# youssefg7/dl-sound-classification

Hardware: AMD Instinct MI355X
Metric: training clips/sec (EnvNet-v2, ESC-50 shape) (higher is better)
Workload: dtype bf16; 1 GPU; EnvNet-v2 train step (BC-mix, fwd, soft-CE, bwd, clip, Adam), ESC-50 shape; global_batch=256, per_gpu_batch=256, clip_samples=220500, parallelism=dp1, model=envnet_v2

## Files before the change

dl-sound-classification_amd/csrc/conv1ch.hip:

```cpp
#include "common.h"

namespace {

constexpr int C1_C = 32, C1_K = 8;
constexpr int C1_BW = 128;
constexpr int C1_SLOTS = C1_BW + C1_K - 1;
constexpr int C1_PSB = 80;
constexpr int C1_HMAX = 64;
constexpr int C1_OLD = C1_BW + 1;
constexpr int C1_LD = (C1_SLOTS * 4 + 255) / 256;

struct C1Args {
  const bf16* dy;
  const float* w;
  bf16* dx;
  int n, oh, ow, h, wd, nchunk;
};

__global__ __launch_bounds__(256) void conv1ch_dgrad_kernel(C1Args g) {
  __shared__ __attribute__((aligned(16))) char rows[2][C1_SLOTS * C1_PSB];
  __shared__ __attribute__((aligned(16))) float outs[C1_HMAX * C1_OLD];
  const int t = threadIdx.x, lane = t & 63, wave = t >> 6;
  const int b = blockIdx.x / g.nchunk;
  const int w0 = (blockIdx.x - b * g.nchunk) * C1_BW;

  for (int i = t; i < C1_HMAX * C1_OLD; i += 256) outs[i] = 0.f;

  bf16x8 bw[16];
  const int ky = lane & 31;
#pragma unroll
  for (int ks = 0; ks < 16; ++ks) {
    const int kx = ks >> 1, co0 = 16 * (ks & 1) + 8 * (lane >> 5);
#pragma unroll
    for (int j = 0; j < 8; ++j)
      bw[ks][j] = ky < C1_K ? (bf16)g.w[((co0 + j) * C1_K + ky) * C1_K + kx] : (bf16)0.f;
  }

  auto slot_of = [](int q, int& s, int& c) __attribute__((always_inline)) {
    const int gq = q >> 3, j = q & 7;
    s = (gq >> 2) * 8 + (gq & 3) + 4 * (j >> 2);
    c = j & 3;
  };
  const bf16* dyb = g.dy + (int64_t)b * g.oh * g.ow * C1_C;
  auto load_row = [&](int r, uint4 (&reg)[C1_LD]) __attribute__((always_inline)) {
    const bf16* src = dyb + (int64_t)r * g.ow * C1_C;
#pragma unroll
    for (int i = 0; i < C1_LD; ++i) {
      int s, c;
      slot_of(t + 256 * i, s, c);
      const int px = w0 - (C1_K - 1) + s;
      uint4 v = make_uint4(0, 0, 0, 0);
      if (r < g.oh && s < C1_SLOTS && px >= 0 && px < g.ow)
        v = *reinterpret_cast<const uint4*>(src + px * C1_C + c * 8);
      reg[i] = v;
    }
  };
  auto store_row = [&](char* dst, const uint4 (&reg)[C1_LD]) __attribute__((always_inline)) {
#pragma unroll
    for (int i = 0; i < C1_LD; ++i) {
      int s, c;
      slot_of(t + 256 * i, s, c);
      if (s < C1_SLOTS) *reinterpret_cast<uint4*>(dst + s * C1_PSB + c * 16) = reg[i];
    }
  };
  const int m = lane & 31, half = lane >> 5;
  auto compute_row = [&](int r) __attribute__((always_inline)) {
    const char* cur = rows[r & 1];
    f32x16 acc;
#pragma unroll
    for (int i = 0; i < 16; ++i) acc[i] = 0.f;
#pragma unroll
    for (int ks = 0; ks < 16; ++ks) {
      const int slot = 32 * wave + m - (ks >> 1) + (C1_K - 1);
      const bf16x8 a = *reinterpret_cast<const bf16x8*>(cur + slot * C1_PSB + (16 * (ks & 1) + 8 * half) * 2);
      acc = __builtin_amdgcn_mfma_f32_32x32x16_bf16(a, bw[ks], acc, 0, 0, 0);
    }
    if (ky < C1_K) {
      float* o = outs + (r + ky) * C1_OLD + 32 * wave + 4 * half;
#pragma unroll
      for (int i = 0; i < 16; ++i) o[(i & 3) + 8 * (i >> 2)] += acc[i];
    }
  };

  uint4 ra[C1_LD], rb[C1_LD];
  load_row(0, ra);
  load_row(1, rb);
  store_row(rows[0], ra);
  __syncthreads();
  for (int r = 0; r < g.oh; r += 2) {
    load_row(r + 2, ra);
    compute_row(r);
    store_row(rows[(r + 1) & 1], rb);
    __syncthreads();
    if (r + 1 >= g.oh) break;
    load_row(r + 3, rb);
    compute_row(r + 1);
    store_row(rows[r & 1], ra);
    __syncthreads();
  }

  bf16* dxb = g.dx + (int64_t)b * g.h * g.wd;
  for (int q = t; q < g.h * (C1_BW / 4); q += 256) {
    const int y = q / (C1_BW / 4), x4 = (q - y * (C1_BW / 4)) * 4;
    const int x = w0 + x4;
    if (x >= g.wd) continue;
    const float* o = outs + y * C1_OLD + x4;
    if (x + 4 <= g.wd) {
      bf16x4 v = {(bf16)o[0], (bf16)o[1], (bf16)o[2], (bf16)o[3]};
      *reinterpret_cast<bf16x4*>(dxb + (int64_t)y * g.wd + x) = v;
    } else {
      for (int i = 0; x + i < g.wd; ++i) dxb[(int64_t)y * g.wd + x + i] = (bf16)o[i];
    }
  }
}

}

extern "C" int mia_conv1ch_dgrad(const void* dy, const float* w, void* dx, int32_t n, int32_t oh, int32_t ow,
                                 mia_stream_t stream) {
  MIA_CHECK_ARG(dy && w && dx && n > 0 && oh > 0 && ow > 0, "conv1ch_dgrad: bad arguments");
  const int h = oh + C1_K - 1, wd = ow + C1_K - 1;
  MIA_CHECK_ARG(h <= C1_HMAX, "conv1ch_dgrad: at most %d output rows (got %d)", C1_HMAX, h);
  MIA_CHECK_ARG(wd % 4 == 0, "conv1ch_dgrad: output width must be a multiple of 4 (got %d)", wd);
  MIA_CHECK_ARG((reinterpret_cast<uintptr_t>(dy) | reinterpret_cast<uintptr_t>(dx)) % 16 == 0,
                "conv1ch_dgrad: dy/dx must be 16-byte aligned");
  MIA_CHECK_ARG((int64_t)oh * ow * C1_C < (1ll << 31), "conv1ch_dgrad: clip too large for 32-bit indexing");
  C1Args a{reinterpret_cast<const bf16*>(dy), w, reinterpret_cast<bf16*>(dx), n, oh, ow, h, wd,
           (int)cdiv(wd, C1_BW)};
  const int64_t blocks = (int64_t)n * a.nchunk;
  MIA_CHECK_ARG(blocks < (1ll << 31), "conv1ch_dgrad: grid too large");
  conv1ch_dgrad_kernel<<<(unsigned)blocks, 256, 0, as_stream(stream)>>>(a);
  MIA_LAUNCH_CHECK("conv1ch_dgrad");
  return 0;
}
```

dl-sound-classification_amd/csrc/dgemm.hip:

```cpp
#include <type_traits>

#include "gemm_common.h"
#include "../../include/miaudio_optim.h"

namespace {

using namespace mgemm;

constexpr int NT = 256;



typedef __attribute__((address_space(3))) void* lds_vp;
typedef const __attribute__((address_space(1))) void* glb_vp;

__device__ __forceinline__ void tile_sqsum_store(double* dst, double v, double* red) {
  v = wave_sum_d(v);
  __syncthreads();
  if ((threadIdx.x & 63) == 0) red[threadIdx.x >> 6] = v;
  __syncthreads();
  if (threadIdx.x == 0) {
    double s = 0.0;
#pragma unroll
    for (int w = 0; w < NT / 64; ++w) s += red[w];
    *dst = s;
  }
}

__global__ __launch_bounds__(NT) void tile_sqsum_kernel(const float* __restrict__ c, int64_t ldc, int64_t M, int64_t N,
                                                        int nbn, double* __restrict__ out) {
  const int bm = blockIdx.x / nbn, bn = blockIdx.x - (blockIdx.x / nbn) * nbn;
  const int64_t m0 = (int64_t)bm * 128, n0 = (int64_t)bn * 128;
  float sq = 0.f;
  for (int e = threadIdx.x; e < 128 * 128; e += NT) {
    const int64_t m = m0 + e / 128, n = n0 + e % 128;
    if (m < M && n < N) {
      const float v = c[m * ldc + n];
      sq = fmaf(v, v, sq);
    }
  }
  __shared__ double red[NT / 64];
  tile_sqsum_store(out + blockIdx.x, (double)sq, red);
}

__device__ __forceinline__ int dkc_swz(int r) { return (r >> 1) & 7; }

template <int L>
struct DLoader {
  const bf16* src[4];
  int64_t step;
  __device__ __forceinline__ void init(const bf16* base, int64_t ld, int64_t rows_or_cols, int64_t r0, int64_t kbeg,
                                       int wave, int lane) {
#pragma unroll
    for (int i = 0; i < 4; ++i) {
      const int j = wave * 4 + i;
      if constexpr (L == MIA_LAYOUT_KC) {
        const int r = 8 * j + (lane >> 3);
        const int c = (lane & 7) ^ dkc_swz(r);
        int64_t row = r0 + r;
        if (row >= rows_or_cols) row = rows_or_cols - 1;
        src[i] = base + row * ld + kbeg + c * 8;
      } else {
        const int kr = 4 * j + (lane >> 4);
        const int p = lane & 15;
        const int c = 2 * ((p >> 1) ^ (kr & 3)) + (p & 1);
        int64_t col = r0 + c * 8;
        if (col + 8 > rows_or_cols) col = rows_or_cols - 8;
        src[i] = base + (kbeg + kr) * ld + col;
      }
    }
    step = L == MIA_LAYOUT_KC ? 64 : 64 * ld;
  }
  __device__ __forceinline__ void issue(char* tile, int wave) {
#pragma unroll
    for (int i = 0; i < 4; ++i) {
      __builtin_amdgcn_global_load_lds((glb_vp)src[i], (lds_vp)(tile + (wave * 4 + i) * 1024), 16, 0, 0);
      src[i] += step;
    }
  }
};

template <int L>
__device__ __forceinline__ bf16x8 dfrag(const char* tile, int rbase, int ks, int lane) {
  if constexpr (L == MIA_LAYOUT_KC) {
    const int rr = rbase + (lane & 31);
    const int c = 2 * ks + (lane >> 5);
    return *reinterpret_cast<const bf16x8*>(tile + rr * 128 + ((c ^ dkc_swz(rr)) * 16));
  } else {
    const int i16 = lane & 15, gq = lane >> 4;
    const int col = rbase + 16 * (gq & 1) + 4 * (i16 & 3);
    const int kr = ks * 16 + 8 * (gq >> 1) + (i16 >> 2);
    const char* p0 = tile + kr * 256 + (((col >> 4) ^ (kr & 3)) * 32) + (col & 15) * 2;
    const s16x4 lo = __builtin_amdgcn_ds_read_tr16_b64_v4i16((MIA_LDS s16x4*)(p0));
    const s16x4 hi = __builtin_amdgcn_ds_read_tr16_b64_v4i16((MIA_LDS s16x4*)(p0 + 4 * 256));
    typedef short s16x8 __attribute__((ext_vector_type(8)));
    const s16x8 cc = {lo[0], lo[1], lo[2], lo[3], hi[0], hi[1], hi[2], hi[3]};
    return __builtin_bit_cast(bf16x8, cc);
  }
}


constexpr int TILE = 128 * 64 * 2;

template <int NS, class R>
__device__ __forceinline__ void dgemm_update_tile(const DArgs& g, const UpdateEpi<R>& o, char* smem) {
  constexpr int L = MIA_LAYOUT_RC;
  const int t = threadIdx.x, lane = t & 63;
  const int wave = __builtin_amdgcn_readfirstlane(t >> 6);
  const int wm = wave >> 1, wn = wave & 1;
  const int nwg = g.nbm * g.nbn;
  const int orig = blockIdx.x;
  const int xcd = orig % 8, q8 = nwg / 8, r8 = nwg % 8;
  const int wgid = (xcd < r8 ? xcd * (q8 + 1) : r8 * (q8 + 1) + (xcd - r8) * q8) + orig / 8;
  const int bm = wgid % g.nbm, bn = wgid / g.nbm;
  const int64_t m0 = (int64_t)bm * 128, n0 = (int64_t)bn * 128;
  const int nk = (int)(g.K / 64);

  DLoader<L> la;
  DLoader<L> lb;
  la.init(g.a, g.lda, g.M, m0, 0, wave, lane);
  lb.init(g.b, g.ldb, g.N, n0, 0, wave, lane);

  f32x16 acc[2][2];
#pragma unroll
  for (int i = 0; i < 2; ++i)
#pragma unroll
    for (int j = 0; j < 2; ++j)
#pragma unroll
      for (int r = 0; r < 16; ++r) acc[i][j][r] = 0.f;

  f32x4 pv[2][4], av[2][4], bv[2][4];
  const int acol = (lane & 31) * 4;
  auto fetch = [&](int it0, int b) {
#pragma unroll
    for (int u = 0; u < 4; ++u) {
      const int64_t off = (m0 + wave * 32 + (it0 + u) * 2 + (lane >> 5)) * o.ld + n0 + acol;
      pv[b][u] = __builtin_nontemporal_load(reinterpret_cast<const f32x4*>(o.p + off));
      if constexpr (NS > 0) av[b][u] = __builtin_nontemporal_load(reinterpret_cast<const f32x4*>(o.s0 + off));
      if constexpr (NS > 1) bv[b][u] = __builtin_nontemporal_load(reinterpret_cast<const f32x4*>(o.s1 + off));
    }
  };
  fetch(0, 0);

  if (nk > 0) {
    la.issue(smem, wave);
    lb.issue(smem + TILE, wave);
  }
  for (int kt = 0; kt < nk; ++kt) {
    char* cur = smem + (kt & 1) * 2 * TILE;
    if (kt + 1 < nk) {
      char* nxt = smem + ((kt + 1) & 1) * 2 * TILE;
      la.issue(nxt, wave);
      lb.issue(nxt + TILE, wave);
      asm volatile("s_waitcnt vmcnt(8)" ::: "memory");
    } else {
      asm volatile("s_waitcnt vmcnt(0)" ::: "memory");
    }
    __builtin_amdgcn_s_barrier();
    const char* As = cur;
    const char* Bs = cur + TILE;
#pragma unroll
    for (int ks = 0; ks < 4; ++ks) {
      bf16x8 fa[2], fb[2];
#pragma unroll
      for (int i = 0; i < 2; ++i) fa[i] = dfrag<L>(As, wm * 64 + i * 32, ks, lane);
#pragma unroll
      for (int j = 0; j < 2; ++j) fb[j] = dfrag<L>(Bs, wn * 64 + j * 32, ks, lane);
#pragma unroll
      for (int i = 0; i < 2; ++i)
#pragma unroll
        for (int j = 0; j < 2; ++j) acc[i][j] = __builtin_amdgcn_mfma_f32_32x32x16_bf16(fa[i], fb[j], acc[i][j], 0, 0, 0);
    }
    asm volatile("s_waitcnt lgkmcnt(0)" ::: "memory");
    __builtin_amdgcn_s_barrier();
  }

  float* tile = reinterpret_cast<float*>(smem);
#pragma unroll
  for (int i = 0; i < 2; ++i)
#pragma unroll
    for (int j = 0; j < 2; ++j)
#pragma unroll
      for (int r = 0; r < 16; ++r) {
        const int row = wm * 64 + i * 32 + (r & 3) + 8 * (r >> 2) + 4 * (lane >> 5);
        const int col = wn * 64 + j * 32 + (lane & 31);
        tile[row * 128 + (col ^ (((row >> 2) & 1) << 5))] = acc[i][j][r];
      }
  __syncthreads();
  const float coef = o.coef[0];
  const bool first = o.first != 0;
#pragma unroll
  for (int grp = 0; grp < 4; ++grp) {
    const int b = grp & 1;
    if (grp + 1 < 4) fetch((grp + 1) * 4, b ^ 1);
#pragma unroll
    for (int u = 0; u < 4; ++u) {
      const int row = wave * 32 + (grp * 4 + u) * 2 + (lane >> 5);
      const int64_t off = (m0 + row) * o.ld + n0 + acol;
      const f32x4 gv = *reinterpret_cast<const f32x4*>(tile + row * 128 + (acol ^ (((row >> 2) & 1) << 5)));
      f32x4 p4 = pv[b][u], a4 = {0.f, 0.f, 0.f, 0.f}, b4 = a4;
      if constexpr (NS > 0) a4 = av[b][u];
      if constexpr (NS > 1) b4 = bv[b][u];
#pragma unroll
      for (int e = 0; e < 4; ++e) {
        float sa = a4[e], sb = b4[e];
        p4[e] = mopt::apply<NS>(o.rule, coef, first, p4[e], gv[e], sa, sb);
        a4[e] = sa;
        b4[e] = sb;
      }
      __builtin_nontemporal_store(p4, reinterpret_cast<f32x4*>(o.p + off));
      if constexpr (NS > 0) __builtin_nontemporal_store(a4, reinterpret_cast<f32x4*>(o.s0 + off));
      if constexpr (NS > 1) __builtin_nontemporal_store(b4, reinterpret_cast<f32x4*>(o.s1 + off));
      if (o.shadow) {
        const bf16x4 h4 = {(bf16)p4[0], (bf16)p4[1], (bf16)p4[2], (bf16)p4[3]};
        __builtin_nontemporal_store(h4, reinterpret_cast<bf16x4*>(o.shadow + off));
      }
    }
  }
}

template <int NS, class R>
__global__ __launch_bounds__(NT) void dgemm_optim_kernel(DArgs g, UpdateEpi<R> o) {
  __shared__ __attribute__((aligned(1024))) char smem[4 * TILE];
  dgemm_update_tile<NS>(g, o, smem);
}

template <int LA, int LB, bool ADAM = false>
__global__ __launch_bounds__(NT) void dgemm_kernel(DArgs g) {
  __shared__ __attribute__((aligned(1024))) char smem[4 * TILE];
  if constexpr (ADAM) {
    dgemm_update_tile<2>(g, g.upd, smem);
    return;
  }
  const int t = threadIdx.x, lane = t & 63;
  const int wave = __builtin_amdgcn_readfirstlane(t >> 6);
  const int wm = wave >> 1, wn = wave & 1;
  const int nwg = g.nbm * g.nbn;
  const int orig = blockIdx.x;
  const int xcd = orig % 8, q8 = nwg / 8, r8 = nwg % 8;
  const int wgid = (xcd < r8 ? xcd * (q8 + 1) : r8 * (q8 + 1) + (xcd - r8) * q8) + orig / 8;
  int bm, bn;
  if (g.nfast) {
    const int gsize = g.gm * g.nbn;
    const int grp = wgid / gsize, rem = wgid - grp * gsize;
    const int gme = min(g.gm, g.nbm - grp * g.gm);
    bm = grp * g.gm + rem % gme;
    bn = rem / gme;
  } else {
    bm = wgid % g.nbm;
    bn = wgid / g.nbm;
  }
  const int64_t m0 = (int64_t)bm * 128, n0 = (int64_t)bn * 128;
  const int z = blockIdx.y;
  const int64_t kbeg = (int64_t)z * g.kper;
  int64_t kend = kbeg + g.kper;
  if (kend > g.K) kend = g.K;
  const int nk = kend > kbeg ? (int)((kend - kbeg) / 64) : 0;

  DLoader<LA> la;
  DLoader<LB> lb;
  la.init(g.a, g.lda, g.M, m0, kbeg, wave, lane);
  lb.init(g.b, g.ldb, g.N, n0, kbeg, wave, lane);

  f32x16 acc[2][2];
#pragma unroll
  for (int i = 0; i < 2; ++i)
#pragma unroll
    for (int j = 0; j < 2; ++j)
#pragma unroll
      for (int r = 0; r < 16; ++r) acc[i][j][r] = 0.f;

  if (nk > 0) {
    la.issue(smem, wave);
    lb.issue(smem + TILE, wave);
  }
  for (int kt = 0; kt < nk; ++kt) {
    char* cur = smem + (kt & 1) * 2 * TILE;
    if (kt + 1 < nk) {
      char* nxt = smem + ((kt + 1) & 1) * 2 * TILE;
      la.issue(nxt, wave);
      lb.issue(nxt + TILE, wave);
      asm volatile("s_waitcnt vmcnt(8)" ::: "memory");
    } else {
      asm volatile("s_waitcnt vmcnt(0)" ::: "memory");
    }
    __builtin_amdgcn_s_barrier();
    const char* As = cur;
    const char* Bs = cur + TILE;
#pragma unroll
    for (int ks = 0; ks < 4; ++ks) {
      bf16x8 fa[2], fb[2];
#pragma unroll
      for (int i = 0; i < 2; ++i) fa[i] = dfrag<LA>(As, wm * 64 + i * 32, ks, lane);
#pragma unroll
      for (int j = 0; j < 2; ++j) fb[j] = dfrag<LB>(Bs, wn * 64 + j * 32, ks, lane);
#pragma unroll
      for (int i = 0; i < 2; ++i)
#pragma unroll
        for (int j = 0; j < 2; ++j) acc[i][j] = __builtin_amdgcn_mfma_f32_32x32x16_bf16(fa[i], fb[j], acc[i][j], 0, 0, 0);
    }
    asm volatile("s_waitcnt lgkmcnt(0)" ::: "memory");
    __builtin_amdgcn_s_barrier();
  }

  const bool plain = g.mode != 0 ||
                     (g.split == 1 && g.e.dtype == MIA_F32 && g.e.act == MIA_ACT_NONE && !g.e.bias &&
                      !g.e.accumulate && !g.e.rm_inner && g.e.alpha == 1.f && m0 + 128 <= g.M && n0 + 128 <= g.N &&
                      (g.e.ldc & 3) == 0 && ((reinterpret_cast<uintptr_t>(g.e.ptr)) & 15) == 0);
  if (plain) {
    float sq = 0.f;
    if (g.e.sqsum) {
#pragma unroll
      for (int i = 0; i < 2; ++i)
#pragma unroll
        for (int j = 0; j < 2; ++j)
#pragma unroll
          for (int r = 0; r < 16; ++r) sq = fmaf(acc[i][j][r], acc[i][j][r], sq);
    }
    if (g.mode == 1) {
      tile_sqsum_store(g.e.sqsum + (int64_t)bm * g.nbn + bn, (double)sq, reinterpret_cast<double*>(smem));
      return;
    }
    float* tile = reinterpret_cast<float*>(smem);
#pragma unroll
    for (int i = 0; i < 2; ++i)
#pragma unroll
      for (int j = 0; j < 2; ++j)
#pragma unroll
        for (int r = 0; r < 16; ++r) {
          const int row = wm * 64 + i * 32 + (r & 3) + 8 * (r >> 2) + 4 * (lane >> 5);
          const int col = wn * 64 + j * 32 + (lane & 31);
          tile[row * 128 + (col ^ (((row >> 2) & 1) << 5))] = acc[i][j][r];
        }
    __syncthreads();
    float* out = reinterpret_cast<float*>(g.e.ptr);
#pragma unroll 4
    for (int it = 0; it < 16; ++it) {
      const int row = wave * 32 + it * 2 + (lane >> 5);
      const int col = (lane & 31) * 4;
      const f32x4 v = *reinterpret_cast<const f32x4*>(tile + row * 128 + (col ^ (((row >> 2) & 1) << 5)));
      __builtin_nontemporal_store(v, reinterpret_cast<f32x4*>(out + (m0 + row) * g.e.ldc + n0 + col));
    }
    if (g.e.sqsum) tile_sqsum_store(g.e.sqsum + (int64_t)bm * g.nbn + bn, (double)sq, reinterpret_cast<double*>(smem));
    return;
  }
  const bool save = g.e.act == MIA_ACT_GELU_SAVE || g.e.act == MIA_ACT_GELU_SAVE_D;
  const bool save_d = g.e.act == MIA_ACT_GELU_SAVE_D;
  const bool drop = g.e.rm_inner && g.e.rm_offset == MIA_RM_DROP && g.e.rm_istride == 1 &&
                    (g.e.act == MIA_ACT_NONE || g.e.act == MIA_ACT_RELU);
  const bool plain16 = g.split == 1 && g.e.dtype == MIA_BF16 &&
                       (g.e.act == MIA_ACT_NONE || g.e.act == MIA_ACT_RELU || g.e.act == MIA_ACT_GELU ||
                        (save && g.e.aux_dtype == MIA_BF16 && (g.e.ldaux & 7) == 0 &&
                         ((reinterpret_cast<uintptr_t>(g.e.aux)) & 15) == 0)) &&
                       !g.e.accumulate && (!g.e.rm_inner || drop) &&
                       g.e.alpha == 1.f && m0 + 128 <= g.M && n0 + 128 <= g.N && (g.e.ldc & 7) == 0 &&
                       ((reinterpret_cast<uintptr_t>(g.e.ptr)) & 15) == 0;
  if (plain16) {
    float* tile = reinterpret_cast<float*>(smem);
#pragma unroll
    for (int i = 0; i < 2; ++i)
#pragma unroll
      for (int j = 0; j < 2; ++j)
#pragma unroll
        for (int r = 0; r < 16; ++r) {
          const int row = wm * 64 + i * 32 + (r & 3) + 8 * (r >> 2) + 4 * (lane >> 5);
          const int col = wn * 64 + j * 32 + (lane & 31);
          tile[row * 128 + (col ^ (((row >> 2) & 1) << 5))] = acc[i][j][r];
        }
    __syncthreads();
    const int col = (lane & 15) * 8;
    float bv[8];
#pragma unroll
    for (int c = 0; c < 8; ++c) bv[c] = g.e.bias ? g.e.bias[n0 + col + c] : 0.f;
    const bool relu = g.e.act == MIA_ACT_RELU, gelu = g.e.act == MIA_ACT_GELU || save;
    bf16* out = reinterpret_cast<bf16*>(g.e.ptr);
    auto pack = [](const float* f) {
      uint32_t w4[4];
#pragma unroll
      for (int q = 0; q < 4; ++q) {
        w4[q] = pk_bf16(f[2 * q], f[2 * q + 1]);
      }
      return make_uint4(w4[0], w4[1], w4[2], w4[3]);
    };
#pragma unroll 4
    for (int it = 0; it < 8; ++it) {
      const int row = wave * 32 + it * 4 + (lane >> 4);
      const int sw = ((row >> 2) & 1) << 5;
      const f32x4 a = *reinterpret_cast<const f32x4*>(tile + row * 128 + (col ^ sw));
      const f32x4 b = *reinterpret_cast<const f32x4*>(tile + row * 128 + ((col + 4) ^ sw));
      float v[8] = {a[0], a[1], a[2], a[3], b[0], b[1], b[2], b[3]};
#pragma unroll
      for (int c = 0; c < 8; ++c) v[c] += bv[c];
      if (save) {
        float d[8];
#pragma unroll
        for (int c = 0; c < 8; ++c) d[c] = save_d ? gelu_erf_grad((float)(bf16)v[c]) : v[c];
        *reinterpret_cast<uint4*>(reinterpret_cast<bf16*>(const_cast<char*>(g.e.aux)) + (m0 + row) * g.e.ldaux +
                                  n0 + col) = pack(d);
      }
#pragma unroll
      for (int c = 0; c < 8; ++c) v[c] = relu ? fmaxf(v[c], 0.f) : (gelu ? gelu_erf(v[c]) : v[c]);
      int64_t prow = m0 + row;
      if (drop) {
        const int64_t x = prow % g.e.rm_inner;
        if (x >= g.e.rm_outer) continue;
        prow = (prow / g.e.rm_inner) * g.e.rm_outer + x;
      }
      *reinterpret_cast<uint4*>(out + prow * g.e.ldc + n0 + col) = pack(v);
    }
    return;
  }

  float* stage = reinterpret_cast<float*>(smem) + wave * (32 * 33);
  double sqg = 0.0;
#pragma unroll
  for (int i = 0; i < 2; ++i)
#pragma unroll
    for (int j = 0; j < 2; ++j) {
#pragma unroll
      for (int r = 0; r < 16; ++r)
        stage[((r & 3) + 8 * (r >> 2) + 4 * (lane >> 5)) * 33 + (lane & 31)] = acc[i][j][r];
      __syncthreads();
      const int row = lane >> 1, c0 = (lane & 1) * 16;
      const int64_t m = m0 + wm * 64 + i * 32 + row;
      const int64_t nb = n0 + wn * 64 + j * 32 + c0;
      if (m < g.M && nb < g.N) {
        float v[16];
#pragma unroll
        for (int c = 0; c < 16; ++c) v[c] = stage[row * 33 + c0 + c];
        if (g.split > 1) {
          float* dst = g.ws + ((int64_t)z * g.M + m) * g.N + nb;
          if (nb + 16 <= g.N && (g.N & 3) == 0) {
#pragma unroll
            for (int q = 0; q < 4; ++q)
              reinterpret_cast<float4*>(dst)[q] = make_float4(v[4 * q], v[4 * q + 1], v[4 * q + 2], v[4 * q + 3]);
          } else {
            for (int c = 0; c < 16; ++c)
              if (nb + c < g.N) dst[c] = v[c];
          }
        } else {
          epi_store16(g.e, m, nb, g.N, v);
          if (g.e.sqsum) {
            float sq = 0.f;
            for (int c = 0; c < 16; ++c)
              if (nb + c < g.N) sq = fmaf(v[c], v[c], sq);
            sqg += sq;
          }
        }
      }
      __syncthreads();
    }
  if (g.e.sqsum && g.split == 1)
    tile_sqsum_store(g.e.sqsum + (int64_t)bm * g.nbn + bn, sqg, reinterpret_cast<double*>(smem));
}

template <int LA, int LB>
hipError_t dgemm_launch2(const DArgs& d, hipStream_t s) {
  dim3 grid((unsigned)(d.nbm * d.nbn), (unsigned)d.split);
  dgemm_kernel<LA, LB><<<grid, NT, 0, s>>>(d);
  return hipGetLastError();
}

hipError_t dgemm_launch(const DArgs& d, int la, int lb, hipStream_t s) {
  if (la == MIA_LAYOUT_KC && lb == MIA_LAYOUT_KC) return dgemm_launch2<MIA_LAYOUT_KC, MIA_LAYOUT_KC>(d, s);
  if (la == MIA_LAYOUT_KC) return dgemm_launch2<MIA_LAYOUT_KC, MIA_LAYOUT_RC>(d, s);
  if (lb == MIA_LAYOUT_KC) return dgemm_launch2<MIA_LAYOUT_RC, MIA_LAYOUT_KC>(d, s);
  return dgemm_launch2<MIA_LAYOUT_RC, MIA_LAYOUT_RC>(d, s);
}

DArgs dgemm_args(const MiaOperand& A, const MiaOperand& B, int64_t M, int64_t N, int64_t K, int split) {
  DArgs d;
  memset(&d, 0, sizeof(d));
  d.a = reinterpret_cast<const bf16*>(A.ptr); d.b = reinterpret_cast<const bf16*>(B.ptr);
  d.lda = A.ld; d.ldb = B.ld; d.M = M; d.N = N; d.K = K;
  d.split = split;
  d.kper = cdiv(cdiv(K, split), 64) * 64;
  d.nbm = (int)cdiv(M, 128); d.nbn = (int)cdiv(N, 128);
  return d;
}

}

namespace mgemm {

bool dgemm_ok(const MiaOperand& A, const MiaOperand& B, int64_t M, int64_t N, int64_t K, int compute) {
  if (compute != MIA_BF16 || K < 64 || K % 64 != 0 || M < 64 || N < 64) return false;
  if (A.kind != MIA_OP_DENSE || B.kind != MIA_OP_DENSE) return false;
  if (A.dtype != MIA_BF16 || B.dtype != MIA_BF16 || A.pre != MIA_PRE_NONE || B.pre != MIA_PRE_NONE) return false;
  if (A.ld % 8 || B.ld % 8 || (reinterpret_cast<uintptr_t>(A.ptr) & 15) || (reinterpret_cast<uintptr_t>(B.ptr) & 15))
    return false;
  if (A.layout == MIA_LAYOUT_KC) { if (A.rows != M || A.cols < K) return false; }
  else { if (A.rows < K || A.cols != M || M % 8) return false; }
  if (B.layout == MIA_LAYOUT_KC) { if (B.rows != N || B.cols < K) return false; }
  else { if (B.rows < K || B.cols != N || N % 8) return false; }
  if (cdiv(M, 128) * cdiv(N, 128) >= (1ll << 31)) return false;
  return true;
}

int dgemm_run(const MiaOperand& A, const MiaOperand& B, const MiaEpilogue& E, int64_t M, int64_t N, int64_t K,
              int split, void* workspace, hipStream_t s) {
  DArgs d = dgemm_args(A, B, M, N, K, split);
  d.nfast = (d.split == 1 && d.nbn <= 32 && d.nbm >= 4 * d.nbn) ? 1 : 0;
  d.gm = (int)std::max<int64_t>(1, std::min<int64_t>(16, (2ll << 20) / (128 * 2 * std::max<int64_t>(K, 64))));
  d.ws = reinterpret_cast<float*>(workspace);
  d.e = to_dev(E);
  hipError_t err = dgemm_launch(d, A.layout, B.layout, s);
  if (err != hipSuccess) return mia::fail(-(int)err, "dgemm launch: %s", hipGetErrorString(err));
  if (d.split > 1) launch_splitk_reduce(d.ws, d.split, M, N, d.e, s);
  return 0;
}

int tile_sqsum_run(const float* c, int64_t ldc, int64_t M, int64_t N, double* sqsum, hipStream_t s) {
  const int64_t nb = mia_gemm_sqsum_slots(M, N);
  MIA_CHECK_ARG(nb < (1ll << 31), "gemm sqsum: too many tiles");
  tile_sqsum_kernel<<<(unsigned)nb, NT, 0, s>>>(c, ldc, M, N, (int)cdiv(N, 128), sqsum);
  MIA_LAUNCH_CHECK("gemm sqsum");
  return 0;
}

}

extern "C" int64_t mia_gemm_sqsum_slots(int64_t M, int64_t N) { return cdiv(M, 128) * cdiv(N, 128); }

static int wgrad_args(const char* who, const MiaOperand* A, const MiaOperand* B, int64_t M, int64_t N, int64_t K,
                      DArgs* d) {
  MIA_CHECK_ARG(A && B, "%s: null descriptor", who);
  MIA_CHECK_ARG(dgemm_ok(*A, *B, M, N, K, MIA_BF16) && M % 128 == 0 && N % 128 == 0,
                "%s: needs bf16 dense operands, M and N multiples of 128, K a multiple of 64", who);
  *d = dgemm_args(*A, *B, M, N, K, 1);
  return 0;
}

extern "C" int mia_gemm_sqsum_only(const MiaOperand* A, const MiaOperand* B, int64_t M, int64_t N, int64_t K,
                                   double* sqsum, mia_stream_t stream) {
  MIA_CHECK_ARG(sqsum, "gemm_sqsum_only: null sqsum");
  DArgs d;
  if (int rc = wgrad_args("gemm_sqsum_only", A, B, M, N, K, &d)) return rc;
  d.nfast = 1; d.gm = 1;
  d.e.dtype = MIA_F32; d.e.alpha = 1.f; d.e.sqsum = sqsum;
  d.mode = 1;
  hipError_t err = dgemm_launch(d, A->layout, B->layout, as_stream(stream));
  if (err != hipSuccess) return mia::fail(-(int)err, "gemm_sqsum_only launch: %s", hipGetErrorString(err));
  return 0;
}

template <int NS, class R>
static int dgemm_update(const char* who, const MiaOperand* A, const MiaOperand* B, int64_t M, int64_t N, int64_t K,
                        const UpdateEpi<R>& o, mia_stream_t stream) {
  DArgs d;
  if (int rc = wgrad_args(who, A, B, M, N, K, &d)) return rc;
  MIA_CHECK_ARG(A->layout == MIA_LAYOUT_RC && B->layout == MIA_LAYOUT_RC, "%s: needs RC operands", who);
  MIA_CHECK_ARG(o.p && o.coef && (NS < 1 || o.s0) && (NS < 2 || o.s1), "%s: null pointer", who);
  MIA_CHECK_ARG(o.ld >= N && o.ld % 4 == 0 &&
                    ((reinterpret_cast<uintptr_t>(o.p) | reinterpret_cast<uintptr_t>(o.s0) |
                      reinterpret_cast<uintptr_t>(o.s1)) & 15) == 0 &&
                    (reinterpret_cast<uintptr_t>(o.shadow) & 7) == 0,
                "%s: parameter and state rows must be 16-B aligned (ld %% 4 == 0), the shadow 8-B aligned", who);
  const dim3 grid((unsigned)(d.nbm * d.nbn));
  hipStream_t s = as_stream(stream);
  if constexpr (std::is_same_v<R, mopt::AdamRule>) {
    d.upd = o;
    dgemm_kernel<MIA_LAYOUT_RC, MIA_LAYOUT_RC, true><<<grid, NT, 0, s>>>(d);
  } else {
    dgemm_optim_kernel<NS><<<grid, NT, 0, s>>>(d, o);
  }
  MIA_LAUNCH_CHECK(who);
  return 0;
}

extern "C" int mia_gemm_adam(const MiaOperand* A, const MiaOperand* B, int64_t M, int64_t N, int64_t K, float* param,
                             float* exp_avg, float* exp_avg_sq, void* shadow_bf16, int64_t ld, const float* coef,
                             float lr_over_bc1, float bc2_sqrt, float beta1, float beta2, float eps, float weight_decay,
                             mia_stream_t stream) {
  const UpdateEpi<mopt::AdamRule> o{param, exp_avg, exp_avg_sq, reinterpret_cast<bf16*>(shadow_bf16), coef, ld, 0,
                                    {lr_over_bc1, bc2_sqrt, beta1, beta2, eps, weight_decay}};
  return dgemm_update<2>("gemm_adam", A, B, M, N, K, o, stream);
}

extern "C" int mia_gemm_adamw(const MiaOperand* A, const MiaOperand* B, int64_t M, int64_t N, int64_t K, float* param,
                              float* exp_avg, float* exp_avg_sq, void* shadow_bf16, int64_t ld, const float* coef,
                              float lr_over_bc1, float bc2_sqrt, float beta1, float beta2, float eps, float lr,
                              float weight_decay, mia_stream_t stream) {
  const UpdateEpi<mopt::AdamWRule> o{param, exp_avg, exp_avg_sq, reinterpret_cast<bf16*>(shadow_bf16), coef, ld, 0,
                                     {lr_over_bc1, bc2_sqrt, beta1, beta2, eps, mopt::adamw_decay(lr, weight_decay)}};
  return dgemm_update<2>("gemm_adamw", A, B, M, N, K, o, stream);
}

extern "C" int mia_gemm_sgd(const MiaOperand* A, const MiaOperand* B, int64_t M, int64_t N, int64_t K, float* param,
                            float* momentum_buf, void* shadow_bf16, int64_t ld, const float* coef, float lr,
                            float momentum, float dampening, float weight_decay, int32_t nesterov, int32_t first_use,
                            mia_stream_t stream) {
  MIA_CHECK_ARG((momentum != 0.f) == (momentum_buf != nullptr), "gemm_sgd: momentum_buf goes with momentum != 0");
  MIA_CHECK_ARG(!nesterov || (momentum > 0.f && dampening == 0.f),
                "gemm_sgd: nesterov needs a momentum and zero dampening");
  const UpdateEpi<mopt::SgdRule> o{param, momentum_buf, nullptr, reinterpret_cast<bf16*>(shadow_bf16), coef, ld,
                                   first_use, mopt::sgd_rule(lr, momentum, dampening, weight_decay, nesterov)};
  return momentum_buf ? dgemm_update<1>("gemm_sgd", A, B, M, N, K, o, stream)
                      : dgemm_update<0>("gemm_sgd", A, B, M, N, K, o, stream);
}
```

Before: 15790 clips/s.

## Add wave-level persistent conv1ch dgrad kernel and streaming split-K dense GEMM

Adds a single-wave persistent kernel for the first-layer conv dgrad. It works on narrow 32-column strips with a 3-deep register prefetch and wave-only barriers, and maps strips across XCDs. This is meant to raise occupancy and remove block-level syncs. It also adds a 512-thread split-K GEMM for small-M KC×KC dense layers, which streams A/B through multi-buffered LDS using global_load_lds and explicit vmcnt waits. Both become the default path, with env var fallbacks, at the cost of extra code paths and more sensitive tuning.

```diff
diff --git a/dl-sound-classification_amd/csrc/conv1ch.hip b/dl-sound-classification_amd/csrc/conv1ch.hip
--- a/dl-sound-classification_amd/csrc/conv1ch.hip
+++ b/dl-sound-classification_amd/csrc/conv1ch.hip
@@ -114,6 +114,130 @@
   }
 }
 
+constexpr int C2_SW = 32;
+constexpr int C2_SLOTS = C2_SW + C1_K - 1;
+constexpr int C2_OLD = C2_SW + 1;
+constexpr int C2_LD = (C2_SLOTS * 4 + 63) / 64;
+constexpr int C2_PF = 3;
+constexpr int C2_WAVES_PER_CU = 12;
+
+struct C2Args {
+  const bf16* dy;
+  const float* w;
+  bf16* dx;
+  int n, oh, ow, h, wd, nstrip, items, nw;
+};
+
+__device__ __forceinline__ void c2_wave_sync() {
+  __builtin_amdgcn_fence(__ATOMIC_RELEASE, "wavefront");
+  __builtin_amdgcn_wave_barrier();
+  __builtin_amdgcn_fence(__ATOMIC_ACQUIRE, "wavefront");
+}
+
+__global__ __launch_bounds__(64) __attribute__((amdgpu_waves_per_eu(3, 4))) void conv1ch_dgrad_wave_kernel(C2Args g) {
+  __shared__ __attribute__((aligned(16))) char row[C2_SLOTS * C1_PSB];
+  __shared__ __attribute__((aligned(16))) float outs[C1_HMAX * C2_OLD];
+  const int lane = threadIdx.x;
+  const int orig = blockIdx.x;
+  const int xcd = orig % 8, q8 = g.nw / 8, r8 = g.nw % 8;
+  const int gw = (xcd < r8 ? xcd * (q8 + 1) : r8 * (q8 + 1) + (xcd - r8) * q8) + orig / 8;
+
+  for (int i = lane; i < C1_HMAX * C2_OLD; i += 64) outs[i] = 0.f;
+
+  bf16x8 bw[16];
+  const int ky = lane & 31;
+#pragma unroll
+  for (int ks = 0; ks < 16; ++ks) {
+    const int kx = ks >> 1, co0 = 16 * (ks & 1) + 8 * (lane >> 5);
+#pragma unroll
+    for (int j = 0; j < 8; ++j) {
+      const float wv = g.w[((co0 + j) * C1_K + (ky & (C1_K - 1))) * C1_K + kx];
+      bw[ks][j] = ky < C1_K ? (bf16)wv : (bf16)0.f;
+    }
+  }
+  auto slot_of = [](int q, int& s, int& c) __attribute__((always_inline)) {
+    const int gq = q >> 3, j = q & 7;
+    s = (gq >> 2) * 8 + (gq & 3) + 4 * (j >> 2);
+    c = j & 3;
+  };
+  const int m = lane & 31, half = lane >> 5;
+
+  for (int item = gw; item < g.items; item += g.nw) {
+    const int b = item / g.nstrip;
+    const int x0 = (item - b * g.nstrip) * C2_SW;
+    const bf16* dyb = g.dy + (int64_t)b * g.oh * g.ow * C1_C;
+    auto load_row = [&](int r, uint4 (&reg)[C2_LD]) __attribute__((always_inline)) {
+      const bf16* src = dyb + (int64_t)min(r, g.oh - 1) * g.ow * C1_C;
+#pragma unroll
+      for (int i = 0; i < C2_LD; ++i) {
+        int s, c;
+        slot_of(lane + 64 * i, s, c);
+        const int px = min(max(x0 - (C1_K - 1) + s, 0), g.ow - 1);
+        reg[i] = *reinterpret_cast<const uint4*>(src + px * C1_C + c * 8);
+      }
+    };
+    auto store_row = [&](const uint4 (&reg)[C2_LD]) __attribute__((always_inline)) {
+#pragma unroll
+      for (int i = 0; i < C2_LD; ++i) {
+        int s, c;
+        slot_of(lane + 64 * i, s, c);
+        const int px = x0 - (C1_K - 1) + s;
+        const uint4 v = px >= 0 && px < g.ow ? reg[i] : make_uint4(0, 0, 0, 0);
+        if (s < C2_SLOTS) *reinterpret_cast<uint4*>(row + s * C1_PSB + c * 16) = v;
+      }
+    };
+    auto compute_row = [&](int r) __attribute__((always_inline)) {
+      f32x16 acc;
+#pragma unroll
+      for (int i = 0; i < 16; ++i) acc[i] = 0.f;
+#pragma unroll
+      for (int ks = 0; ks < 16; ++ks) {
+        const int slot = m - (ks >> 1) + (C1_K - 1);
+        const bf16x8 a = *reinterpret_cast<const bf16x8*>(row + slot * C1_PSB + (16 * (ks & 1) + 8 * half) * 2);
+        acc = __builtin_amdgcn_mfma_f32_32x32x16_bf16(a, bw[ks], acc, 0, 0, 0);
+      }
+      if (ky < C1_K) {
+        float* o = outs + (r + ky) * C2_OLD + 4 * half;
+#pragma unroll
+        for (int i = 0; i < 16; ++i) o[(i & 3) + 8 * (i >> 2)] += acc[i];
+      }
+    };
+
+    uint4 rg[C2_PF][C2_LD];
+#pragma unroll
+    for (int u = 0; u < C2_PF; ++u) {
+      load_row(u, rg[u]);
+      __builtin_amdgcn_sched_barrier(0);
+    }
+    for (int r0 = 0; r0 < g.oh; r0 += C2_PF) {
+#pragma unroll
+      for (int u = 0; u < C2_PF; ++u) {
+        const int r = r0 + u;
+        if (r < g.oh) store_row(rg[u]);
+        load_row(r + C2_PF, rg[u]);
+        if (r < g.oh) {
+          c2_wave_sync();
+          compute_row(r);
+          c2_wave_sync();
+        }
+      }
+    }
+
+    bf16* dxb = g.dx + (int64_t)b * g.h * g.wd;
+    for (int q = lane; q < g.h * (C2_SW / 4); q += 64) {
+      const int y = q / (C2_SW / 4), x4 = (q - y * (C2_SW / 4)) * 4;
+      const int x = x0 + x4;
+      float* o = outs + y * C2_OLD + x4;
+      const bf16x4 v = {(bf16)o[0], (bf16)o[1], (bf16)o[2], (bf16)o[3]};
+      o[0] = 0.f; o[1] = 0.f; o[2] = 0.f; o[3] = 0.f;
+      if (x + 4 <= g.wd) *reinterpret_cast<bf16x4*>(dxb + (int64_t)y * g.wd + x) = v;
+    }
+    c2_wave_sync();
+  }
+}
+
+bool conv1ch_v1() { const char* e = getenv("MIA_CONV1CH_V1"); return e && e[0] == '1'; }
+
 }
 
 extern "C" int mia_conv1ch_dgrad(const void* dy, const float* w, void* dx, int32_t n, int32_t oh, int32_t ow,
@@ -125,6 +249,17 @@
   MIA_CHECK_ARG((reinterpret_cast<uintptr_t>(dy) | reinterpret_cast<uintptr_t>(dx)) % 16 == 0,
                 "conv1ch_dgrad: dy/dx must be 16-byte aligned");
   MIA_CHECK_ARG((int64_t)oh * ow * C1_C < (1ll << 31), "conv1ch_dgrad: clip too large for 32-bit indexing");
+  if (!conv1ch_v1()) {
+    const int64_t nstrip = cdiv(wd, C2_SW), items = (int64_t)n * nstrip;
+    MIA_CHECK_ARG(items < (1ll << 30), "conv1ch_dgrad: too many column strips");
+    const int64_t slots = (int64_t)mia::cu_count() * C2_WAVES_PER_CU;
+    const int64_t nw = cdiv(items, cdiv(items, slots));
+    C2Args a{reinterpret_cast<const bf16*>(dy), w, reinterpret_cast<bf16*>(dx), n, oh, ow, h, wd,
+             (int)nstrip, (int)items, (int)nw};
+    conv1ch_dgrad_wave_kernel<<<(unsigned)nw, 64, 0, as_stream(stream)>>>(a);
+    MIA_LAUNCH_CHECK("conv1ch_dgrad");
+    return 0;
+  }
   C1Args a{reinterpret_cast<const bf16*>(dy), w, reinterpret_cast<bf16*>(dx), n, oh, ow, h, wd,
            (int)cdiv(wd, C1_BW)};
   const int64_t blocks = (int64_t)n * a.nchunk;
diff --git a/dl-sound-classification_amd/csrc/dgemm.hip b/dl-sound-classification_amd/csrc/dgemm.hip
--- a/dl-sound-classification_amd/csrc/dgemm.hip
+++ b/dl-sound-classification_amd/csrc/dgemm.hip
@@ -454,6 +454,132 @@
     tile_sqsum_store(g.e.sqsum + (int64_t)bm * g.nbn + bn, sqg, reinterpret_cast<double*>(smem));
 }
 
+constexpr int SNT = 512;
+constexpr int S_ADEPTH = 3, S_BDEPTH = 4;
+constexpr int S_LDS = (2 * S_ADEPTH + S_BDEPTH) * TILE;
+
+template <int NI>
+struct SLoader {
+  const bf16* src[NI];
+  int j0;
+  __device__ __forceinline__ void init(const bf16* base, int64_t ld, int64_t rows, int64_t r0, int64_t kbeg, int j0_,
+                                       int lane) {
+    j0 = j0_;
+#pragma unroll
+    for (int i = 0; i < NI; ++i) {
+      const int r = 8 * (j0 + i) + (lane >> 3);
+      const int c = (lane & 7) ^ dkc_swz(r);
+      int64_t row = r0 + r;
+      if (row >= rows) row = rows - 1;
+      src[i] = base + row * ld + kbeg + c * 8;
+    }
+  }
+  __device__ __forceinline__ void issue(char* tile) {
+#pragma unroll
+    for (int i = 0; i < NI; ++i) {
+      __builtin_amdgcn_global_load_lds((glb_vp)src[i], (lds_vp)(tile + (j0 + i) * 1024), 16, 0, 0);
+      src[i] += 64;
+    }
+  }
+};
+
+__global__ __launch_bounds__(SNT) void dgemm_stream_kernel(DArgs g) {
+  constexpr int L = MIA_LAYOUT_KC;
+  __shared__ __attribute__((aligned(1024))) char smem[S_LDS];
+  const int t = threadIdx.x, lane = t & 63;
+  const int wave = __builtin_amdgcn_readfirstlane(t >> 6);
+  const int mb = wave >> 2, wm = (wave >> 1) & 1, wn = wave & 1;
+  const int nwg = g.nbn * g.split;
+  const int orig = blockIdx.x;
+  const int xcd = orig % 8, q8 = nwg / 8, r8 = nwg % 8;
+  const int wgid = (xcd < r8 ? xcd * (q8 + 1) : r8 * (q8 + 1) + (xcd - r8) * q8) + orig / 8;
+  const int z = wgid / g.nbn, bn = wgid - z * g.nbn;
+  const int64_t n0 = (int64_t)bn * 128;
+  const int64_t kbeg = (int64_t)z * g.kper;
+  int64_t kend = kbeg + g.kper;
+  if (kend > g.K) kend = g.K;
+  const int nk = kend > kbeg ? (int)((kend - kbeg) / 64) : 0;
+  const bool live = (int64_t)mb * 128 < g.M;
+
+  SLoader<4> la;
+  SLoader<2> lb;
+  la.init(g.a, g.lda, g.M, (int64_t)mb * 128, kbeg, (wave & 3) * 4, lane);
+  lb.init(g.b, g.ldb, g.N, n0, kbeg, wave * 2, lane);
+
+  f32x16 acc[2][2];
+#pragma unroll
+  for (int i = 0; i < 2; ++i)
+#pragma unroll
+    for (int j = 0; j < 2; ++j)
+#pragma unroll
+      for (int r = 0; r < 16; ++r) acc[i][j][r] = 0.f;
+
+  char* const abase = smem + mb * TILE;
+  char* const bbase = smem + 2 * S_ADEPTH * TILE;
+  int ia = 0, ib = 0;
+  auto push_a = [&]() __attribute__((always_inline)) {
+    la.issue(abase + ia * 2 * TILE);
+    ia = ia + 1 == S_ADEPTH ? 0 : ia + 1;
+  };
+  auto push_b = [&]() __attribute__((always_inline)) {
+    lb.issue(bbase + ib * TILE);
+    ib = ib + 1 == S_BDEPTH ? 0 : ib + 1;
+  };
+  if (nk > 0) { push_a(); push_b(); }
+  if (nk > 1) { push_a(); push_b(); }
+  if (nk > 2) push_b();
+  int ca = 0, cb = 0;
+  for (int kt = 0; kt < nk; ++kt) {
+    const int rem = nk - 1 - kt;
+    if (rem >= 2) asm volatile("s_waitcnt vmcnt(8)" ::: "memory");
+    else if (rem == 1) asm volatile("s_waitcnt vmcnt(6)" ::: "memory");
+    else asm volatile("s_waitcnt vmcnt(0)" ::: "memory");
+    __builtin_amdgcn_s_barrier();
+    if (kt + 2 < nk) push_a();
+    if (kt + 3 < nk) push_b();
+    if (live) {
+      const char* As = abase + ca * 2 * TILE;
+      const char* Bs = bbase + cb * TILE;
+#pragma unroll
+      for (int ks = 0; ks < 4; ++ks) {
+        bf16x8 fa[2], fb[2];
+#pragma unroll
+        for (int i = 0; i < 2; ++i) fa[i] = dfrag<L>(As, wm * 64 + i * 32, ks, lane);
+#pragma unroll
+        for (int j = 0; j < 2; ++j) fb[j] = dfrag<L>(Bs, wn * 64 + j * 32, ks, lane);
+#pragma unroll
+        for (int i = 0; i < 2; ++i)
+#pragma unroll
+          for (int j = 0; j < 2; ++j)
+            acc[i][j] = __builtin_amdgcn_mfma_f32_32x32x16_bf16(fa[i], fb[j], acc[i][j], 0, 0, 0);
+      }
+    }
+    ca = ca + 1 == S_ADEPTH ? 0 : ca + 1;
+    cb = cb + 1 == S_BDEPTH ? 0 : cb + 1;
+    asm volatile("s_waitcnt lgkmcnt(0)" ::: "memory");
+  }
+
+  if (live) {
+#pragma unroll
+    for (int i = 0; i < 2; ++i)
+#pragma unroll
+      for (int j = 0; j < 2; ++j)
+#pragma unroll
+        for (int r = 0; r < 16; ++r) {
+          const int64_t m = (int64_t)mb * 128 + wm * 64 + i * 32 + (r & 3) + 8 * (r >> 2) + 4 * (lane >> 5);
+          const int64_t n = n0 + wn * 64 + j * 32 + (lane & 31);
+          if (m < g.M) g.ws[((int64_t)z * g.M + m) * g.N + n] = acc[i][j][r];
+        }
+  }
+}
+
+bool dense_v1() { const char* e = getenv("MIA_DENSE_V1"); return e && e[0] == '1'; }
+
+bool dgemm_stream_ok(const DArgs& d, int la, int lb) {
+  return la == MIA_LAYOUT_KC && lb == MIA_LAYOUT_KC && d.M <= 256 && d.N % 128 == 0 && d.split >= 2 &&
+         d.kper >= 3 * 64 && (int64_t)d.nbn * d.split < (1ll << 31);
+}
+
 template <int LA, int LB>
 hipError_t dgemm_launch2(const DArgs& d, hipStream_t s) {
   dim3 grid((unsigned)(d.nbm * d.nbn), (unsigned)d.split);
@@ -504,7 +630,13 @@
   d.gm = (int)std::max<int64_t>(1, std::min<int64_t>(16, (2ll << 20) / (128 * 2 * std::max<int64_t>(K, 64))));
   d.ws = reinterpret_cast<float*>(workspace);
   d.e = to_dev(E);
-  hipError_t err = dgemm_launch(d, A.layout, B.layout, s);
+  hipError_t err;
+  if (!dense_v1() && dgemm_stream_ok(d, A.layout, B.layout)) {
+    dgemm_stream_kernel<<<(unsigned)(d.nbn * d.split), SNT, 0, s>>>(d);
+    err = hipGetLastError();
+  } else {
+    err = dgemm_launch(d, A.layout, B.layout, s);
+  }
   if (err != hipSuccess) return mia::fail(-(int)err, "dgemm launch: %s", hipGetErrorString(err));
   if (d.split > 1) launch_splitk_reduce(d.ws, d.split, M, N, d.e, s);
   return 0;
```

New measurement: 15900 clips/s (median of 6 runs). Within noise of the previous version (+0.7%).
